# cvg/nice-slam

Measured on AMD Instinct MI355X. Metric: rendered rays/sec (fwd+bwd) per mapping iter, higher is better.
Workload: dtype f32 (f64 sample placement / depth)

## Files before the change

nice_slam_amd/build.py:

```python
from __future__ import annotations

import os
import shutil
import subprocess

HERE = os.path.dirname(os.path.abspath(__file__))
CSRC = os.path.join(HERE, "csrc")
OUT = os.path.join(HERE, "libnsr.so")
SOURCES = ("nsr_api.cpp",)
HEADERS = ("nsr_kernels.h", "nsr_recon.h", "nsr_meshdist.h", "nsr_bound.h", "nsr_raster.h", "nsr_view.h", "nsr_imgmetrics.h", "nsr_figure.h", "nsr_frame.h", "nsr_pose.h", "nsr_trajeval.h", "nsr_jpeg.h", "nsr_jpegdec.h", "nsr_bwd2.h", "nsr_fwd2.h", "nsr_layout.h", "nsr_dev.h", "nsr_rt.h", os.path.join("..", "..", "include", "nsr.h"))
FLAGS = ("--offload-arch=gfx950", "-O3", "-std=c++17", "-ffp-contract=off", "-munsafe-fp-atomics",
         "-fPIC", "-shared", "-x", "hip")


def hipcc_path() -> str:
    for cand in (os.environ.get("HIPCC"), shutil.which("hipcc"), "/opt/rocm/bin/hipcc"):
        if cand and os.path.exists(cand):
            return cand
    raise RuntimeError("hipcc not found: cannot build libnsr.so")


STAMP = os.path.join(HERE, "libnsr.srchash")


def source_hash() -> str:
    import hashlib
    h = hashlib.sha256(" ".join(FLAGS).encode())
    for f in SOURCES + HEADERS:
        with open(os.path.join(CSRC, f), "rb") as fh:
            h.update(f.encode() + b"\0" + fh.read())
    return h.hexdigest()


def is_fresh() -> bool:
    if not os.path.exists(OUT) or not os.path.exists(STAMP):
        return False
    try:
        with open(STAMP) as f:
            return f.read().strip() == source_hash()
    except OSError:
        return False


def build_lib(force: bool = False, verbose: bool = False) -> str:
    if not force and is_fresh():
        return OUT
    stamp = source_hash()
    cmd = [hipcc_path(), *FLAGS, "-Rpass-analysis=kernel-resource-usage", *[os.path.join(CSRC, s) for s in SOURCES], "-o", OUT]
    if verbose:
        print(" ".join(cmd))
    res = subprocess.run(cmd, capture_output=True, text=True)
    if res.returncode != 0:
        raise RuntimeError("hipcc failed:\n" + res.stdout + res.stderr)
    _write_resources(res.stderr)
    with open(STAMP, "w") as f:
        f.write(stamp + "\n")
    return OUT


RESOURCES = os.path.join(HERE, "libnsr.resources.json")


def _write_resources(remarks: str):
    import json
    import re
    out, name = {}, None
    for line in remarks.splitlines():
        m = re.search(r"Function Name: (\S+)", line)
        if m:
            name = m.group(1)
            out[name] = {}
            continue
        for key, pat in (("vgprs", r" VGPRs: (\d+)"), ("agprs", r"AGPRs: (\d+)"), ("scratch_bytes_per_lane", r"ScratchSize \[bytes/lane\]: (\d+)"),
                         ("sgprs", r"TotalSGPRs: (\d+)"), ("occupancy_waves_per_simd", r"Occupancy \[waves/SIMD\]: (\d+)")):
            m = re.search(pat, line)
            if m and name:
                out[name][key] = int(m.group(1))
    with open(RESOURCES, "w") as f:
        json.dump(out, f, indent=1, sort_keys=True)


if __name__ == "__main__":
    print(build_lib(force=True, verbose=True))
```

nice_slam_amd/csrc/nsr_api.cpp:

```cpp
#include <cmath>
#include <cstdio>
#include <cstdlib>
#include <cstring>
#include <map>
#include <mutex>
#include <string>
#include <utility>

#include "nsr_rt.h"
#include "nsr_kernels.h"
#include "../../nice_slam_amd/csrc/nsr_recon.h"
#include "../../nice_slam_amd/csrc/nsr_meshdist.h"
#include "../../nice_slam_amd/csrc/nsr_bound.h"
#include "../../nice_slam_amd/csrc/nsr_raster.h"
#include "../../nice_slam_amd/csrc/nsr_view.h"
#include "../../nice_slam_amd/csrc/nsr_imgmetrics.h"
#include "../../nice_slam_amd/csrc/nsr_figure.h"
#include "../../nice_slam_amd/csrc/nsr_frame.h"
#include "../../nice_slam_amd/csrc/nsr_pose.h"
#include "../../nice_slam_amd/csrc/nsr_trajeval.h"
#include "../../nice_slam_amd/csrc/nsr_jpeg.h"
#include "../../nice_slam_amd/csrc/nsr_jpegdec.h"

namespace {
// ... 127 lines not shown
    for (int s = first; s <= last; ++s) {
        const nsr_grid &g = a->grid[s];
        if (!g.feat) return fail("nsr: missing feature grid for this stage");
        if (g.Z < 1 || g.Y < 1 || g.X < 1) return fail("nsr: bad grid shape");
        if ((long long)g.Z * g.Y * g.X >= (1ll << 25)) return fail("nsr: grid too large for 32-bit byte offsets (2^25 voxels = 4 GB)");
        nsr::GridDev &G = P.grid[s];
        G.feat = g.feat; G.dfeat = g.dfeat; G.gmask = a->grad_voxel_mask[s]; G.Z = g.Z; G.Y = g.Y; G.X = g.X;
        for (int i = 0; i < 3; ++i) {
            if (!(g.hi[i] > g.lo[i])) return fail("nsr: empty normalisation box");
            G.lo[i] = g.lo[i];
            G.ext[i] = g.hi[i] - g.lo[i];
            G.inv[i] = 1.0 / (g.hi[i] - g.lo[i]);
        }
        const nsr_decoder &d = a->dec[s];
        if (!d.params || !d.packed) return fail("nsr: missing decoder parameters / packed stream for this stage");
        P.dec[s].params = d.params; P.dec[s].packed = d.packed; P.dec[s].dparams = d.dparams;
    }
    P.depth = a->depth; P.var = a->var; P.rgb = a->rgb; P.raw = a->raw; P.zvals = a->zvals;
    P.gt_color = a->gt_color; P.keep = a->keep; P.loss = a->loss; P.w_color = a->w_color;
    P.skip_masked = (a->skip_masked && a->keep && a->acts && a->zvals && a->raw) ? 1 : 0;
    P.dl_depth = a->dl_depth; P.dl_rgb = a->dl_rgb; P.loss_depth = a->gt_depth;
    return 0;
}

int finish(const char *what) {
    if (const char *e = nsr::rt_check_last()) return fail(std::string(what) + ": " + e);
    return 0;
}

template <typename K>
int launch_cfg(K kernel, int lds_bytes, const char *what) {
    if (lds_bytes > kLdsLimit) return fail(std::string(what) + ": LDS budget exceeded");
    if (lds_bytes <= 48 * 1024) return 0;
    static std::mutex mu;
    static std::map<std::pair<const void *, int>, int> granted;
    const std::pair<const void *, int> key(reinterpret_cast<const void *>(kernel), nsr::rt_current_device());
    std::lock_guard<std::mutex> lock(mu);
    int &g = granted[key];
    if (lds_bytes > g) {
        if (const char *e = nsr::rt_allow_lds(kernel, lds_bytes)) return fail(std::string(what) + ": " + e);
        g = lds_bytes;
    }
    return 0;
}

int fwd_lds_bytes(int stage, int npts) {
    const int wl = stage == NSR_STAGE_COARSE ? nsr::packed_total(0) : (stage == NSR_STAGE_MIDDLE ? nsr::packed_total(1) : nsr::packed_total(2));
    return round16(3 * nsr::AUX_FLOATS * 4) + npts * (8 + 8 + 16) + wl * 4;
}

int render_bwd_split(const nsr_render_args *a, const nsr_bwd_args *b, nsr::RenderParams &P, bool any_params, void *stream) {
    const SplitLayout L = split_layout(P.stage, P.n_rays, P.S);
    if (L.stride * 4 >= (1ll << 31)) return fail("nsr_render_bwd: more than 2^25 sample points in one call (split the ray batch)");
    const SplitGeo G = split_geo(P.stage, P.n_rays, P.S, b->max_blocks);
    const int passes = bwd_passes(P.stage);
    P.dy = P.acts + L.o_dy;
    P.draw = P.acts + L.o_draw;
    P.pf = P.acts + L.o_pf;
    P.pd = reinterpret_cast<double *>(P.acts + L.o_pd);
    for (int s = 0; s < 4; ++s)
        if (P.dec[s].dparams && (P.acts_masks_only & (1 | (2 << (s == NSR_COARSE ? 0 : s - NSR_MIDDLE)))))
            return fail("nsr_render_bwd: the forward saved relu masks only for a decoder whose parameter gradients are asked for (acts_masks_only); they need the full activations");
    if (P.dec[NSR_FINE].dparams && (P.acts_masks_only & (1 | 2)))
        return fail("nsr_render_bwd: the forward saved relu masks only for the middle decoder (acts_masks_only), whose features the fine decoder's parameter gradients read");
    if (any_params) {
        const long long need = (long long)passes * ((long long)G.nimg * P.partial_stride + (long long)G.nb * nsr::kDbPart);
        if (!b->workspace || b->workspace_floats < need) return fail("nsr_render_bwd: workspace too small");
        P.partials = b->workspace;
        P.dbpart = b->workspace + (long long)passes * G.nimg * P.partial_stride;
    }
    if (b->ev_start) nsr::rt_record(b->ev_start, stream);
    const bool draw_ready = b->loss_grads_from_forward && a->loss && a->dl_depth && b->d_depth == a->dl_depth && !b->d_var &&
                            (b->d_rgb == nullptr || b->d_rgb == a->dl_rgb) && (P.stage != NSR_STAGE_COLOR || b->d_rgb == a->dl_rgb || !a->gt_color);
    P.draw_scaled = draw_ready ? 0 : 1;
    if (!draw_ready) {
        const int tb = 256, rays_per_block = tb / 64;
        NSR_LAUNCH(nsr::comp_bwd_kernel, dim3((unsigned)((P.n_rays + rays_per_block - 1) / rays_per_block)), dim3(tb), 0, stream, P);
    }
    const bool rays = P.d_rays_o != nullptr;
    {
        int lds = 0;
        const int first = P.stage == NSR_STAGE_COARSE ? NSR_COARSE : NSR_MIDDLE, last = P.stage == NSR_STAGE_COARSE ? NSR_COARSE : P.stage;
        for (int kind = first; kind <= last; ++kind) {
            const int need = (nsr::AUX_FLOATS + nsr::packedT_total(kind) + G.waves * nsr::kDxStg + 4) * 4;
            lds = need > lds ? need : lds;
        }
        P.hot_slots = 0;
        if (P.stage != NSR_STAGE_COARSE) {
            int slots = (kLdsLimit - lds) / (nsr::kHotRow * 4);
            slots = slots > kHotSlotCap ? kHotSlotCap : slots;
            P.hot_slots = slots < 16 ? 16 : slots;
            lds += P.hot_slots * nsr::kHotRow * 4;
        }
        for (int s = 0; s < 4; ++s) {
            P.hot_z[s] = 0.f;
            if (s == NSR_COARSE || kHotCells <= 0 || !P.grid[s].dfeat) continue;
            double cell = 0.0;
            const int nn[3] = {P.grid[s].X, P.grid[s].Y, P.grid[s].Z};
            for (int ax = 0; ax < 3; ++ax) { const double c = nn[ax] > 1 ? P.grid[s].ext[ax] / (nn[ax] - 1) : 0.0; cell = c > cell ? c : cell; }
            P.hot_z[s] = (float)(kHotCells * cell);
        }
        P.lds_grid_floats = 0;
        if (P.stage == NSR_STAGE_COARSE && P.grid[NSR_COARSE].dfeat) {
            const long long gf = (long long)P.grid[NSR_COARSE].X * P.grid[NSR_COARSE].Y * P.grid[NSR_COARSE].Z * nsr::kC;
            if (lds + gf * 4 <= kLdsLimit) { P.lds_grid_floats = (int)gf; lds += (int)gf * 4; }
        }
        {
            const long long tiles = (P.n_points_total + nsr::kTile - 1) / nsr::kTile;
            int wgt[3] = {0, 0, 0}, wsum = 0;
            for (int p = 0; p < passes; ++p) {
                const int s = P.stage == NSR_STAGE_COARSE ? NSR_COARSE : NSR_MIDDLE + p;
                wgt[p] = (P.dec[s].dparams || rays || P.stage == NSR_STAGE_COARSE) ? kDxFullWeight : kDxLightWeight;
                wsum += wgt[p];
            }
            const int total = passes * G.nb;
            int used = 0;
            P.dx_beg[0] = 0;
            for (int p = 0; p < 3; ++p) {
                long long n = 0;
                if (p < passes) {
                    n = p == passes - 1 ? total - used : (long long)total * wgt[p] / wsum;
                    if (n < 1) n = 1;
                    if (n > tiles) n = tiles;
                }
                used += (int)n;
                P.dx_beg[p + 1] = P.dx_beg[p] + (int)n;
            }
        }
        const dim3 grid(P.dx_beg[3]), block(64 * G.waves);
#define NSR_DX(ST, RY)                                                                                  \
    if (int rc = launch_cfg(nsr::render_bwd_dx_kernel<ST, RY>, lds, "nsr_render_bwd(dx)")) return rc;   \
    NSR_LAUNCH((nsr::render_bwd_dx_kernel<ST, RY>), grid, block, lds, stream, P);
        switch (P.stage) {
            case 0: if (rays) { NSR_DX(0, true) } else { NSR_DX(0, false) } break;
            case 1: if (rays) { NSR_DX(1, true) } else { NSR_DX(1, false) } break;
            case 2: if (rays) { NSR_DX(2, true) } else { NSR_DX(2, false) } break;
            default: if (rays) { NSR_DX(3, true) } else { NSR_DX(3, false) } break;
        }
#undef NSR_DX
    }
    if (b->ev_dx_done) nsr::rt_record(b->ev_dx_done, stream);
    if (any_params) {
        const int lds = nsr::dw_lds_bytes(P.stage >= NSR_STAGE_FINE ? NSR_FINE : NSR_MIDDLE);
        const long long tiles = (P.n_points_total + nsr::kTile - 1) / nsr::kTile;
        int wgt[3] = {0, 0, 0}, wsum = 0;
        for (int p = 0; p < passes; ++p) {
            const int s = P.stage == NSR_STAGE_COARSE ? NSR_COARSE : NSR_MIDDLE + p;
            wgt[p] = P.dec[s].dparams ? (s == NSR_FINE ? dw_fine_weight(P.stage) : kDwWeight) : 0;
            wsum += wgt[p];
        }
        const int total = passes * G.nimg;
        P.dw_beg[0] = 0;
        for (int p = 0; p < 3; ++p) {
            long long n = (p < passes && wgt[p]) ? (long long)total * wgt[p] / wsum : 0;
            if (p < passes && wgt[p] && n < 1) n = 1;
            if (n > tiles) n = tiles;
            P.dw_beg[p + 1] = P.dw_beg[p] + (int)n;
        }
        const dim3 grid(P.dw_beg[3]), block(64 * nsr::kDwWaves);
#define NSR_DW(ST)                                                                                  \
    if (int rc = launch_cfg(nsr::render_bwd_dw_kernel<ST>, lds, "nsr_render_bwd(dw)")) return rc;   \
    NSR_LAUNCH((nsr::render_bwd_dw_kernel<ST>), grid, block, lds, stream, P);
        switch (P.stage) {
            case 0: NSR_DW(0) break;
            case 1: NSR_DW(1) break;
            case 2: NSR_DW(2) break;
            default: NSR_DW(3) break;
// ... 1987 lines not shown
```

nice_slam_amd/csrc/nsr_bwd2.h:

```cpp
#pragma once

namespace nsr {

constexpr int kDySlots = 10;
constexpr int kDxMaxWaves = 12;
constexpr int kDxTx = 0, kDxTab = kTile * kTxS, kDxP = kDxTab + 256, kDxDP = kDxP + 48, kDxStg = kDxDP + 48;
static_assert(kDxStg % 4 == 0, "staging regions must stay 16-byte aligned");
constexpr int kDbPart = 288;
NSR_KERNEL void comp_bwd_kernel(const RenderParams P) {
    const int lane = tid() & 63, wave = tid() >> 6, nw = nthreads() >> 6;
    const long long ray = (long long)bid_x() * nw + wave;
    if (ray >= P.n_rays) return;
    const int S = P.S;
    if (!ray_live(P, ray)) {
        if (lane < S) st4(P.draw + (ray * S + lane) * 4, F4{0.f, 0.f, 0.f, 0.f});
        return;
    }
    const bool act = lane < S;
    const long long gp = ray * S + (act ? lane : 0);
    const F4 rw = act ? ld4(P.raw + gp * 4) : F4{0.f, 0.f, 0.f, 0.f};
    const double sc = P.g_scale ? P.g_scale[0] : 1.0;
    const double gD = P.d_depth ? P.d_depth[ray] * sc : 0.0, gV = P.d_var ? P.d_var[ray] * sc : 0.0, dep = P.g_depth[ray];
    float gr = 0.f, gg = 0.f, gb = 0.f;
    if (P.d_rgb) { gr = P.d_rgb[ray * 3 + 0] * (float)sc; gg = P.d_rgb[ray * 3 + 1] * (float)sc; gb = P.d_rgb[ray * 3 + 2] * (float)sc; }
    const double z = act ? P.zvals[gp] : 0.0;
    const Comp cw = comp_weights(rw.w, act, lane);
    const double dz = z - dep;
    const double s1 = wave_sum_d((double)cw.w * dz);
    const float Gz = (float)(gD * z + gV * (dz * dz - 2.0 * s1 * z));
    const float Gw = Gz + fmaf(gb, rw.z, fmaf(gg, rw.y, gr * rw.x));
    float v = act ? Gw * cw.w : 0.f;
#pragma unroll
    for (int d = 1; d < 64; d <<= 1) {
        const float o = shfl_down(v, d);
        if (lane + d < 64) v += o;
    }
    float suffix = shfl_down(v, 1);
    if (lane == 63) suffix = 0.f;
    const float dalpha = Gw * cw.T - suffix / cw.t;
    float docc = 10.f * (dalpha * ((1.f - cw.alpha) * cw.alpha));
    const double px = (double)P.rays_o[ray * 3 + 0] + (double)P.rays_d[ray * 3 + 0] * z;
    const double py = (double)P.rays_o[ray * 3 + 1] + (double)P.rays_d[ray * 3 + 1] * z;
    const double pz = (double)P.rays_o[ray * 3 + 2] + (double)P.rays_d[ray * 3 + 2] * z;
    const bool inside = (px > P.blo[0]) && (px < P.bhi[0]) && (py > P.blo[1]) && (py < P.bhi[1]) && (pz > P.blo[2]) && (pz < P.bhi[2]);
    if (!inside) docc = 0.f;
    if (act) {
        st4(P.draw + gp * 4, F4{cw.w * gr, cw.w * gg, cw.w * gb, docc});
        double *q = P.pd + gp * 4;
        q[0] = px; q[1] = py; q[2] = pz; q[3] = z;
        st4(P.pf + gp * 4, F4{(float)px, (float)py, (float)pz, 0.f});
    }
}

template <int NTK>
NSR_DEV void gemv_t(f32x4 (&dx)[NTK], const Act<2> &dy, const float *wt, int lane) {
#pragma unroll
    for (int To = 0; To < 2; ++To) {
        f32x4 a[NTK];
#pragma unroll
        for (int Tk = 0; Tk < NTK; ++Tk) a[Tk] = to_v(ld4(wt + ((Tk * 2 + To) * 64 + lane) * 4));
#pragma unroll
        for (int r = 0; r < 4; ++r)
#pragma unroll
            for (int Tk = 0; Tk < NTK; ++Tk) dx[Tk] = mfma16(a[Tk][r], dy.t[To][r], dx[Tk]);
    }
    sched_fence();
}

struct DxIn {
    F4 dr;
    unsigned m0, m1;
};
NSR_DEV DxIn dx_load(const RenderParams &P, const float *acts_pass, long long tile, int pt, int g) {
    DxIn I;
    const long long gp = tile * kTile + pt;
    const long long q = gp < P.n_points_total ? gp : 0;
    I.dr = ld4(P.draw + q * 4);
    const float *mp = acts_pass + ((q >> 4) * kActSlots + kActMask) * 256 + ((q & 15) * 4 + g) * 4;
    I.m0 = __builtin_bit_cast(unsigned, mp[0]);
    I.m1 = __builtin_bit_cast(unsigned, mp[1]);
    return I;
}
NSR_DEV void dx_keep(const DxIn &I) {
    keep_alive(I.dr.w); keep_alive(__builtin_bit_cast(float, I.m1));
}

template <int KIND, bool PARAMS, bool RAYS>
NSR_DEV void dx_pass(const RenderParams &P, int bi, int nbp, int gb) {
    constexpr bool XYZ = KIND != NSR_COARSE;
    constexpr int NOUT = nout_of(KIND);
    char *lds = lds_base();
    const int lane = tid() & 63, wave = uniform(tid() >> 6), nw = nthreads() >> 6;
    const int pt = lane & 15, g = lane >> 4;
    float *aux = reinterpret_cast<float *>(lds);
    float *wt = aux + AUX_FLOATS;
    float *stg = wt + packedT_total(KIND);
    float *Sw = stg + wave * kDxStg;
    const int tail_off = uniform((int)(stg + nw * kDxStg - reinterpret_cast<float *>(lds)));
    const int gl_off = (KIND == NSR_COARSE && P.lds_grid_floats > 0) ? tail_off : -1;
    float *gl = gl_off >= 0 ? reinterpret_cast<float *>(lds) + gl_off : nullptr;
    const bool use_hot = KIND != NSR_COARSE && P.hot_z[KIND] > 0.f && P.grid[KIND].dfeat != nullptr;
    const HotTab hot{use_hot ? tail_off : -1, P.hot_slots};
    int *tcnt = reinterpret_cast<int *>(stg + nw * kDxStg + (KIND == NSR_COARSE ? P.lds_grid_floats : P.hot_slots * kHotRow));
    const GridDev &G = P.grid[KIND];
    const DecDev &D = P.dec[KIND];
    const bool do_grid = G.dfeat != nullptr;
    if (!do_grid && !PARAMS && !RAYS) return;
    const Dbg dbg{P.dbg ? P.dbg + ((long long)gb * kDxMaxWaves + wave) * 64 : nullptr};
    dbg.stamp(0);
    constexpr long long sstride = 256;
    const float *acts_pass = P.acts + (long long)act_pass(KIND) * P.act_tiles * kActSlots * 256;
    const long long ntiles = (P.n_points_total + kTile - 1) / kTile;
    const long long t0 = ntiles * bi / nbp, tend = ntiles * (bi + 1) / nbp;
    long long tile = t0 + wave;
    const bool pre = tile < tend && tile_live(P, tile);
    DxIn cur;
    if (pre) cur = dx_load(P, acts_pass, tile, pt, g);
    copy_f4<AUX_FLOATS / 4>(aux, D.packed);
    copy_f4_dma<packedT_total(KIND) / 4>(wt, D.packed + AUX_FLOATS + packed_total(KIND));
    if (gl) for (int i = tid(); i < P.lds_grid_floats; i += nthreads()) gl[i] = 0.f;
    if (use_hot) hot_init(hot);
    if (tid() == 0) tcnt[0] = nw;
    dma_wait<0>();
    block_sync();
    dbg.stamp(1);
    float *dys = P.dy + (long long)act_pass(KIND) * P.act_tiles * kDySlots * 256;
    const bool need_dc = do_grid || RAYS;
    float aB[kET][3];
#pragma unroll
    for (int k = 0; k < kET; ++k) { aB[k][0] = 0.f; aB[k][1] = 0.f; aB[k][2] = 0.f; }

    auto claim = [&]() -> long long {
        for (;;) {
            int k = 0;
            if (lane == 0) k = atomic_fetch_add_lds_i(tcnt, 1);
            const long long t = t0 + shfl_i(k, 0);
            if (t >= tend || tile_live(P, t)) return t;
        }
    };
    const float dr_scale = (!P.draw_scaled && P.g_scale) ? (float)P.g_scale[0] : 1.f;
    if (!pre) {
        tile = claim();
        if (tile < tend) cur = dx_load(P, acts_pass, tile, pt, g);
    }
    if (tile < tend) dx_keep(cur);
    while (tile < tend) {
        loop_fence();
        const long long nxt = claim();
        const bool has_next = nxt < tend;
        DxIn nx = cur;
        if (has_next) nx = dx_load(P, acts_pass, nxt, pt, g);
        const long long gp = tile * kTile + pt;
        const bool active = gp < P.n_points_total;
        const double *pp = P.pd + (active ? gp : 0) * 4;
        const double cpx = pp[0], cpy = pp[1], cpz = pp[2], cz = pp[3];
        dbg.stamp(2);
        const unsigned mw0 = active ? cur.m0 : 0u, mw1 = active ? cur.m1 : 0u;
        const float dsc = active ? dr_scale : 0.f;
        float d_out[4] = {0.f, 0.f, 0.f, 0.f};
        if (NOUT == 1) d_out[0] = cur.dr.w * dsc;
        else { d_out[0] = cur.dr.x * dsc; d_out[1] = cur.dr.y * dsc; d_out[2] = cur.dr.z * dsc; }
        Act<2> dh;
#pragma unroll
        for (int T = 0; T < 2; ++T) {
            f32x4 v = f4zero();
#pragma unroll
            for (int n = 0; n < (NOUT == 1 ? 1 : 3); ++n) {
                const F4 w = ld4(aux + AUX_WO + n * 32 + 16 * T + 4 * g);
                v[0] = fmaf(w.x, d_out[n], v[0]); v[1] = fmaf(w.y, d_out[n], v[1]);
                v[2] = fmaf(w.z, d_out[n], v[2]); v[3] = fmaf(w.w, d_out[n], v[3]);
            }
            dh.t[T] = v;
        }
        Act<2> dc, dY0, dY3;
        act_zero(dc); act_zero(dY0); act_zero(dY3);
        float *dyp = dys + tile * (kDySlots * 256) + (pt * 4 + g) * 4;
#pragma unroll
        for (int I = 4; I >= 0; --I) {
            if (XYZ && need_dc) gemv_t<2>(dc.t, dh, wt + xyzT_u(I), lane);
            const Act<2> dY = apply_mask(dh, I < 4 ? mw0 : mw1, I < 4 ? 8 * I : 0);
            if (PARAMS && active) {
                st4(dyp + (2 * I) * sstride, to_F4(dY.t[0]));
                st4(dyp + (2 * I + 1) * sstride, to_F4(dY.t[1]));
            }
            if (I == 3) dY3 = dY;
            if (I == 0) dY0 = dY;
            if (!XYZ) {
                if (I == 3 && need_dc) gemv_t<2>(dc.t, dY, wt + nox_mat(NW3C).pk, lane);
                if (I == 0 && need_dc) gemv_t<2>(dc.t, dY, wt + nox_mat(NW0).pk, lane);
            }
            if (I > 0) {
                Act<2> nd;
                act_zero(nd);
                if (XYZ) gemv_t<2>(nd.t, dY, wt + xyzT_wh(I - 1), lane);
                else gemv_t<2>(nd.t, dY, wt + nox_mat(I == 1 ? NW1 : (I == 2 ? NW2 : (I == 3 ? NW3H : NW4))).pk, lane);
                dh = nd;
            }
        }
        dbg.stamp(3);
        const float px = (float)cpx, py = (float)cpy, pz = (float)cpz;
        float dpe[3] = {0.f, 0.f, 0.f};
        if (XYZ && PARAMS && ballot64(active) != 0ull) {
            if (g == 0) { Sw[kDxP + pt] = px; Sw[kDxP + 16 + pt] = py; Sw[kDxP + 32 + pt] = pz; }
            wave_fence();
            const f32x4 qx = to_v(ld4(Sw + kDxP + 4 * g)), qy = to_v(ld4(Sw + kDxP + 16 + 4 * g)), qz = to_v(ld4(Sw + kDxP + 32 + 4 * g));
            f32x4 sx = f4zero(), sy = f4zero(), sz = f4zero();
#pragma unroll
            for (int Tk = 0; Tk < kET; ++Tk) {
                f32x4 e0 = f4zero(), e3 = f4zero();
#pragma unroll
                for (int To = 0; To < 2; ++To) {
                    const f32x4 a0 = to_v(ld4(wt + xyzT_w0() + ((Tk * 2 + To) * 64 + lane) * 4));
                    const f32x4 a3 = to_v(ld4(wt + xyzT_w3e() + ((Tk * 2 + To) * 64 + lane) * 4));
#pragma unroll
                    for (int r = 0; r < 4; ++r) {
                        e0 = mfma16(dY0.t[To][r], a0[r], e0);
                        e3 = mfma16(dY3.t[To][r], a3[r], e3);
                    }
                }
                sched_fence();
                const F4 b = load_b1(aux, 16 * Tk + pt);
                const f32x4 darg = (e0 + e3) * cos_dx4(vfma(qz, splat(b.z), vfma(qy, splat(b.y), qx * splat(b.x))));
#pragma unroll
                for (int r = 0; r < 4; ++r) {
                    aB[Tk][0] = fmaf(darg[r], qx[r], aB[Tk][0]); aB[Tk][1] = fmaf(darg[r], qy[r], aB[Tk][1]);
                    aB[Tk][2] = fmaf(darg[r], qz[r], aB[Tk][2]);
                }
                if (RAYS) { sx = vfma(darg, splat(b.x), sx); sy = vfma(darg, splat(b.y), sy); sz = vfma(darg, splat(b.z), sz); }
            }
            if (RAYS) {
#pragma unroll
                for (int m = 1; m < 16; m <<= 1)
#pragma unroll
                    for (int r = 0; r < 4; ++r) { sx[r] += shfl_xor(sx[r], m); sy[r] += shfl_xor(sy[r], m); sz[r] += shfl_xor(sz[r], m); }
                if (pt == 0) { st4(Sw + kDxDP + 4 * g, to_F4(sx)); st4(Sw + kDxDP + 16 + 4 * g, to_F4(sy)); st4(Sw + kDxDP + 32 + 4 * g, to_F4(sz)); }
                wave_fence();
                dpe[0] = Sw[kDxDP + pt]; dpe[1] = Sw[kDxDP + 16 + pt]; dpe[2] = Sw[kDxDP + 32 + pt];
            }
            wave_fence();
        } else if (XYZ && RAYS) {
            f32x4 dE[kET];
#pragma unroll
            for (int Tk = 0; Tk < kET; ++Tk) dE[Tk] = f4zero();
            gemv_t<kET>(dE, dY0, wt + xyzT_w0(), lane);
            gemv_t<kET>(dE, dY3, wt + xyzT_w3e(), lane);
            float ax = 0.f, ay = 0.f, az = 0.f;
#pragma unroll
            for (int Tk = 0; Tk < kET; ++Tk) {
                const B4 b = load_b4(aux, 4 * Tk + g);
                const f32x4 darg = dE[Tk] * cos_dx4(vfma(splat(pz), b.z, vfma(splat(py), b.y, splat(px) * b.x)));
#pragma unroll
                for (int r = 0; r < 4; ++r) { ax = fmaf(darg[r], b.x[r], ax); ay = fmaf(darg[r], b.y[r], ay); az = fmaf(darg[r], b.z[r], az); }
                sched_fence();
            }
            dpe[0] = red_g(ax); dpe[1] = red_g(ay); dpe[2] = red_g(az);
        }
        dbg.stamp(4);
        Lvl L;
        if (need_dc) L = make_level(G, cpx, cpy, cpz);
        const unsigned live = (do_grid && G.gmask) ? gmask_bits(G, L, g) : 3u;
        float dux = 0.f, duy = 0.f, duz = 0.f;
        if (RAYS) coord_grad(G, L, g, dc, dux, duy, duz);
        dx_keep(nx);
        keep_alive_d(cpx); keep_alive_d(cpy); keep_alive_d(cpz); keep_alive_d(cz);
        dbg.stamp(5);
        if (do_grid)
            scatter_merged(G, L, lane, dc, active, Sw + kDxTx, Sw + kDxTab, gl_off, hot, (float)cz < P.hot_z[KIND], live);
        dbg.stamp(6);
        if (RAYS) {
            double v[6];
            const bool mine = active && g == 0;
            v[0] = mine ? (double)dux * (2.0 * G.inv[0]) + (double)dpe[0] : 0.0;
            v[1] = mine ? (double)duy * (2.0 * G.inv[1]) + (double)dpe[1] : 0.0;
            v[2] = mine ? (double)duz * (2.0 * G.inv[2]) + (double)dpe[2] : 0.0;
            v[3] = v[0] * cz; v[4] = v[1] * cz; v[5] = v[2] * cz;
            if ((P.S & (kTile - 1)) == 0) {
#pragma unroll
                for (int m = 1; m < 16; m <<= 1)
#pragma unroll
                    for (int q = 0; q < 6; ++q) v[q] += shfl_xor_d(v[q], m);
                if (lane == 0 && active) {
                    const long long ray = (long long)((unsigned)gp / (unsigned)P.S);
#pragma unroll
                    for (int q = 0; q < 3; ++q) {
                        atomic_add_global(P.d_rays_o + ray * 3 + q, (float)v[q]);
                        atomic_add_global(P.d_rays_d + ray * 3 + q, (float)v[3 + q]);
                    }
                }
            } else if (mine) {
                const long long ray = (long long)((unsigned)gp / (unsigned)P.S);
#pragma unroll
                for (int q = 0; q < 3; ++q) {
                    atomic_add_global(P.d_rays_o + ray * 3 + q, (float)v[q]);
                    atomic_add_global(P.d_rays_d + ray * 3 + q, (float)v[3 + q]);
                }
            }
        }
        cur = nx;
        tile = nxt;
        dbg.stamp(7);
    }
    dbg.stamp(8);
    if (XYZ && PARAMS) {
#pragma unroll
        for (int k = 0; k < kET; ++k)
#pragma unroll
            for (int d = 0; d < 3; ++d) {
                float v = aB[k][d];
                v += shfl_xor(v, 16); v += shfl_xor(v, 32);
                if (g == 0) Sw[d * 96 + 16 * k + pt] = v;
            }
    }
    if (use_hot || (gl && do_grid) || (XYZ && PARAMS)) block_sync();
    dbg.stamp(10);
    if (XYZ && PARAMS) {
        float *part = P.dbpart + (long long)gb * kDbPart;
        for (int t = tid(); t < kDbPart; t += nthreads()) {
            float s = 0.f;
            for (int w = 0; w < nw; ++w) s += stg[w * kDxStg + t];
            part[t] = s;
        }
    }
    if (use_hot) hot_flush(hot, G);
    dbg.stamp(11);
    if (gl && do_grid) {
        for (int i = tid(); i < P.lds_grid_floats; i += nthreads()) {
            const float v = gl[i];
            if (v != 0.f) atomic_add_global(G.dfeat + i, v);
// ... 595 lines not shown
```

nice_slam_amd/csrc/nsr_kernels.h:

```cpp
#pragma once
#include "nsr_dev.h"
#include "nsr_layout.h"
#include "../../include/nsr.h"

namespace nsr {

template <int NT>
struct Act { f32x4 t[NT]; };

NSR_DEV f32x4 f4zero() { f32x4 v = {0.f, 0.f, 0.f, 0.f}; return v; }
NSR_DEV f32x4 to_v(F4 a) { f32x4 v = {a.x, a.y, a.z, a.w}; return v; }
NSR_DEV F4 to_F4(f32x4 v) { return F4{v[0], v[1], v[2], v[3]}; }
template <int NT> NSR_DEV void act_zero(Act<NT> &a) {
#pragma unroll
    for (int T = 0; T < NT; ++T) a.t[T] = f4zero();
}

NSR_DEV double tmax(double a, double b) { return (a > b || a != a) ? a : b; }
NSR_DEV double tmin(double a, double b) { return (a < b || a != a) ? a : b; }

struct GridDev {
    const float *feat;
    float *dfeat;
    const unsigned char *gmask;
    int Z, Y, X;
    double lo[3];
    double ext[3];
    double inv[3];
};

struct DecDev {
    const float *params;
    const float *packed;
    float *dparams;
};

struct RenderParams {
    int stage, n_samples, n_surface, S;
    long long n_rays;
    int rays_per_block, tiles_per_block;
    long long n_groups;
    const float *rays_o, *rays_d, *gt_depth, *gt_max;
    double blo[3], bhi[3];
    float t_uniform[NSR_MAX_SAMPLES];
    double t_surface[NSR_MAX_SAMPLES];
    GridDev grid[4];
    DecDev dec[4];
    double *depth, *var;
    float *rgb, *raw;
    double *zvals;
    float *acts;
    int acts_masks_only;
    long long n_points_total;
    long long act_tiles;
    const double *d_depth, *d_var, *g_depth;
    const double *g_scale;
    const float *d_rgb;
    float *d_rays_o, *d_rays_d;
    float *partials;
    int partial_stride;
    const float *loss_depth;
    const float *gt_color;
    const unsigned char *keep;
    double *loss;
    double *dl_depth;
    float *dl_rgb;
    float w_color;
    long long *dbg;
    float *dy;
    float *draw;
    double *pd;
    float *pf;
    float *dbpart;
    int dw_beg[4];
    int dx_beg[4];
    int draw_scaled;
    int skip_masked;
    int lds_grid_floats;
    float hot_z[4];
    int hot_slots;
    unsigned s_magic;
    int pass_beg[4];
    const double *points;
    long long n_points;
    float *out_points;
// ... 1979 lines not shown
```

nice_slam_amd/csrc/nsr_layout.h:

```cpp
#pragma once

namespace nsr {

constexpr int kC = 32;
constexpr int kH = 32;
constexpr int kE = 93;
constexpr int kET = 6;
constexpr int kTile = 16;
constexpr int kTxS = 36;

struct Mat {
    int off;
    int stride;
    int kbeg;
    int kcols;
    int nt;
    int pk;
};

constexpr int cdim_of(int kind) { return kind == 2 ? 64 : 32; }
constexpr int nout_of(int kind) { return kind == 3 ? 4 : 1; }
constexpr bool is_xyz(int kind) { return kind != 0; }

constexpr int xyz_fcw(int cd, int i) { return i * (32 * cd + 32); }
// ... 17 lines not shown
}
constexpr int xyz_pk(int cd, int id) {
    int o = 0;
    for (int j = 0; j < id; ++j) o += xyz_nt(cd, j) * 512;
    return o;
}
constexpr Mat xyz_mat(int cd, int id) {
    switch (id) {
        case XW0: return Mat{xyz_w(cd, 0), kE, 0, kE, kET, xyz_pk(cd, id)};
        case XU0: return Mat{xyz_fcw(cd, 0), cd, 0, cd, cd / 16, xyz_pk(cd, id)};
        case XW1: return Mat{xyz_w(cd, 1), 32, 0, 32, 2, xyz_pk(cd, id)};
        case XU1: return Mat{xyz_fcw(cd, 1), cd, 0, cd, cd / 16, xyz_pk(cd, id)};
        case XW2: return Mat{xyz_w(cd, 2), 32, 0, 32, 2, xyz_pk(cd, id)};
        case XU2: return Mat{xyz_fcw(cd, 2), cd, 0, cd, cd / 16, xyz_pk(cd, id)};
        case XW3E: return Mat{xyz_w(cd, 3), kE + 32, 0, kE, kET, xyz_pk(cd, id)};
        case XW3H: return Mat{xyz_w(cd, 3), kE + 32, kE, 32, 2, xyz_pk(cd, id)};
        case XU3: return Mat{xyz_fcw(cd, 3), cd, 0, cd, cd / 16, xyz_pk(cd, id)};
        case XW4: return Mat{xyz_w(cd, 4), 32, 0, 32, 2, xyz_pk(cd, id)};
        default: return Mat{xyz_fcw(cd, 4), cd, 0, cd, cd / 16, xyz_pk(cd, id)};
    }
}
constexpr int xyz_packed_total(int cd) { return xyz_pk(cd, XNMAT); }

constexpr int nox_in(int i) { return i == 3 ? 64 : 32; }
constexpr int nox_w(int i) {
    int o = 0;
    for (int j = 0; j < i; ++j) o += 32 * nox_in(j) + 32;
    return o;
}
constexpr int nox_b(int i) { return nox_w(i) + 32 * nox_in(i); }
constexpr int nox_wo() { return nox_b(4) + 32; }
constexpr int nox_bo() { return nox_wo() + 32; }
constexpr int nox_total() { return nox_bo() + 1; }
enum { NW0 = 0, NW1 = 1, NW2 = 2, NW3C = 3, NW3H = 4, NW4 = 5, NNMAT = 6 };
constexpr Mat nox_mat(int id) {
    switch (id) {
        case NW0: return Mat{nox_w(0), 32, 0, 32, 2, 0};
        case NW1: return Mat{nox_w(1), 32, 0, 32, 2, 1024};
        case NW2: return Mat{nox_w(2), 32, 0, 32, 2, 2048};
        case NW3C: return Mat{nox_w(3), 64, 0, 32, 2, 3072};
        case NW3H: return Mat{nox_w(3), 64, 32, 32, 2, 4096};
        default: return Mat{nox_w(4), 32, 0, 32, 2, 5120};
    }
}
constexpr int nox_packed_total() { return 6144; }

constexpr int param_total(int kind) { return kind == 0 ? nox_total() : xyz_total(cdim_of(kind), nout_of(kind)); }
constexpr int packed_total(int kind) { return kind == 0 ? nox_packed_total() : xyz_packed_total(cdim_of(kind)); }
constexpr int nmat_of(int kind) { return kind == 0 ? (int)NNMAT : (int)XNMAT; }
constexpr Mat mat_of(int kind, int id) { return kind == 0 ? nox_mat(id) : xyz_mat(cdim_of(kind), id); }
constexpr int bias_off(int kind, int i) { return kind == 0 ? nox_b(i) : xyz_b(cdim_of(kind), i); }
constexpr int fcb_off(int kind, int i) { return xyz_fcb(cdim_of(kind), i); }
constexpr int wo_off(int kind) { return kind == 0 ? nox_wo() : xyz_wo(cdim_of(kind)); }
constexpr int bo_off(int kind) { return kind == 0 ? nox_bo() : xyz_bo(cdim_of(kind), nout_of(kind)); }
constexpr int B_off(int kind) { return xyz_B(cdim_of(kind)); }

static_assert(param_total(0) == 6337, "coarse decoder parameter count");
static_assert(param_total(1) == 15800, "middle decoder parameter count");
static_assert(param_total(2) == 20920, "fine decoder parameter count");
static_assert(param_total(3) == 15899, "color decoder parameter count");

constexpr int AUX_B = 0;
constexpr int AUX_V = 160;
constexpr int AUX_WO = 320;
constexpr int AUX_BO = 448;
constexpr int AUX_BM = 452;
constexpr int AUX_FLOATS = 452 + 96 * 4;
constexpr int xyzT_u(int i) { return i * 1024; }
constexpr int xyzT_wh(int m) { return 5120 + m * 1024; }
constexpr int xyzT_w0() { return 9216; }
constexpr int xyzT_w3e() { return 12288; }
constexpr int xyzT_total() { return 15360; }
constexpr int packedT_total(int kind) { return kind == 0 ? nox_packed_total() : xyzT_total(); }
constexpr int xyzT_nmat() { return 11; }
constexpr Mat xyzT_mat(int cd, int id) {
    return id < 5 ? Mat{xyz_fcw(cd, id), cd, 0, 32, 2, xyzT_u(id)}
         : id == 5 ? Mat{xyz_w(cd, 1), 32, 0, 32, 2, xyzT_wh(0)}
         : id == 6 ? Mat{xyz_w(cd, 2), 32, 0, 32, 2, xyzT_wh(1)}
         : id == 7 ? Mat{xyz_w(cd, 3), kE + 32, kE, 32, 2, xyzT_wh(2)}
         : id == 8 ? Mat{xyz_w(cd, 4), 32, 0, 32, 2, xyzT_wh(3)}
         : id == 9 ? Mat{xyz_w(cd, 0), kE, 0, kE, kET, xyzT_w0()}
                   : Mat{xyz_w(cd, 3), kE + 32, 0, kE, kET, xyzT_w3e()};
}
constexpr int nmatT_of(int kind) { return kind == 0 ? (int)NNMAT : xyzT_nmat(); }
constexpr Mat matT_of(int kind, int id) { return kind == 0 ? nox_mat(id) : xyzT_mat(cdim_of(kind), id); }

constexpr int packed_buf_total(int kind) { return AUX_FLOATS + packed_total(kind) + packedT_total(kind); }
static_assert(AUX_FLOATS % 4 == 0, "the operand stream behind the aux table must stay 16-byte aligned");

}
```

Measured before the change: 4.758 million.

## Use split-bf16 MFMA for embedding-gradient products in dx backward

```diff
diff --git a/nice_slam_amd/build.py b/nice_slam_amd/build.py
--- a/nice_slam_amd/build.py
+++ b/nice_slam_amd/build.py
@@ -8,7 +8,7 @@
 CSRC = os.path.join(HERE, "csrc")
 OUT = os.path.join(HERE, "libnsr.so")
 SOURCES = ("nsr_api.cpp",)
-HEADERS = ("nsr_kernels.h", "nsr_recon.h", "nsr_meshdist.h", "nsr_bound.h", "nsr_raster.h", "nsr_view.h", "nsr_imgmetrics.h", "nsr_figure.h", "nsr_frame.h", "nsr_pose.h", "nsr_trajeval.h", "nsr_jpeg.h", "nsr_jpegdec.h", "nsr_bwd2.h", "nsr_fwd2.h", "nsr_layout.h", "nsr_dev.h", "nsr_rt.h", os.path.join("..", "..", "include", "nsr.h"))
+HEADERS = ("nsr_kernels.h", "nsr_recon.h", "nsr_meshdist.h", "nsr_bound.h", "nsr_raster.h", "nsr_view.h", "nsr_imgmetrics.h", "nsr_figure.h", "nsr_frame.h", "nsr_pose.h", "nsr_trajeval.h", "nsr_jpeg.h", "nsr_jpegdec.h", "nsr_bwd2.h", "nsr_fwd2.h", "nsr_layout.h", "nsr_split.h", "nsr_dev.h", "nsr_rt.h", os.path.join("..", "..", "include", "nsr.h"))
 FLAGS = ("--offload-arch=gfx950", "-O3", "-std=c++17", "-ffp-contract=off", "-munsafe-fp-atomics",
          "-fPIC", "-shared", "-x", "hip")
 
diff --git a/nice_slam_amd/csrc/nsr_api.cpp b/nice_slam_amd/csrc/nsr_api.cpp
--- a/nice_slam_amd/csrc/nsr_api.cpp
+++ b/nice_slam_amd/csrc/nsr_api.cpp
@@ -233,7 +233,7 @@
         int lds = 0;
         const int first = P.stage == NSR_STAGE_COARSE ? NSR_COARSE : NSR_MIDDLE, last = P.stage == NSR_STAGE_COARSE ? NSR_COARSE : P.stage;
         for (int kind = first; kind <= last; ++kind) {
-            const int need = (nsr::AUX_FLOATS + nsr::packedT_total(kind) + G.waves * nsr::kDxStg + 4) * 4;
+            const int need = (nsr::AUX_FLOATS + nsr::dx_stream_lds(kind) + G.waves * nsr::kDxStg + 4) * 4;
             lds = need > lds ? need : lds;
         }
         P.hot_slots = 0;
diff --git a/nice_slam_amd/csrc/nsr_bwd2.h b/nice_slam_amd/csrc/nsr_bwd2.h
--- a/nice_slam_amd/csrc/nsr_bwd2.h
+++ b/nice_slam_amd/csrc/nsr_bwd2.h
@@ -66,6 +66,19 @@
     }
     sched_fence();
 }
+NSR_DEV bf16x8w ld_plane(const float *p) {
+    const F4 v = ld4(p);
+    bf16x8w w = {__builtin_bit_cast(unsigned, v.x), __builtin_bit_cast(unsigned, v.y), __builtin_bit_cast(unsigned, v.z), __builtin_bit_cast(unsigned, v.w)};
+    return w;
+}
+NSR_DEV void st_plane(float *p, bf16x8w w) {
+    const unsigned w0 = w[0], w1 = w[1], w2 = w[2], w3 = w[3];
+    st4(p, F4{__builtin_bit_cast(float, w0), __builtin_bit_cast(float, w1), __builtin_bit_cast(float, w2), __builtin_bit_cast(float, w3)});
+}
+NSR_DEV Bf3 ld_planes(const float *planes, int Tk, int lane) {
+    const float *p = planes + (Tk * 3 * 64 + lane) * 4;
+    return Bf3{ld_plane(p), ld_plane(p + 256), ld_plane(p + 512)};
+}
 
 struct DxIn {
     F4 dr;
@@ -94,7 +107,7 @@
     const int pt = lane & 15, g = lane >> 4;
     float *aux = reinterpret_cast<float *>(lds);
     float *wt = aux + AUX_FLOATS;
-    float *stg = wt + packedT_total(KIND);
+    float *stg = wt + dx_stream_lds(KIND);
     float *Sw = stg + wave * kDxStg;
     const int tail_off = uniform((int)(stg + nw * kDxStg - reinterpret_cast<float *>(lds)));
     const int gl_off = (KIND == NSR_COARSE && P.lds_grid_floats > 0) ? tail_off : -1;
@@ -116,11 +129,27 @@
     const bool pre = tile < tend && tile_live(P, tile);
     DxIn cur;
     if (pre) cur = dx_load(P, acts_pass, tile, pt, g);
+    const float *streamT = D.packed + AUX_FLOATS + packed_total(KIND);
+    constexpr bool EMB = XYZ && (PARAMS || RAYS);
+    constexpr int kPlaneJobs = 2 * kET * 64;
+    int pj = tid();
+    F4 pv0 = F4{0.f, 0.f, 0.f, 0.f}, pv1 = pv0;
+    auto plane_src = [&](int j) { return streamT + (j >= kET * 64 ? xyzT_w3e() : xyzT_w0()) + (((j >> 6) % kET) * 128 + (j & 63)) * 4; };
+    if (EMB && pj < kPlaneJobs) { pv0 = ld4(plane_src(pj)); pv1 = ld4(plane_src(pj) + 256); }
     copy_f4<AUX_FLOATS / 4>(aux, D.packed);
-    copy_f4_dma<packedT_total(KIND) / 4>(wt, D.packed + AUX_FLOATS + packed_total(KIND));
+    copy_f4_dma<(XYZ ? xyzT_copied() : packedT_total(KIND)) / 4>(wt, streamT);
     if (gl) for (int i = tid(); i < P.lds_grid_floats; i += nthreads()) gl[i] = 0.f;
     if (use_hot) hot_init(hot);
     if (tid() == 0) tcnt[0] = nw;
+    if (EMB) {
+        while (pj < kPlaneJobs) {
+            const Bf3 s = split_pack8(to_v(pv0), to_v(pv1));
+            float *dst = wt + xyzL_planes(pj >= kET * 64 ? 1 : 0) + (((pj >> 6) % kET) * 3 * 64 + (pj & 63)) * 4;
+            st_plane(dst, s.hi); st_plane(dst + 256, s.mid); st_plane(dst + 512, s.lo);
+            pj += nthreads();
+            if (pj < kPlaneJobs) { pv0 = ld4(plane_src(pj)); pv1 = ld4(plane_src(pj) + 256); }
+        }
+    }
     dma_wait<0>();
     block_sync();
     dbg.stamp(1);
@@ -203,22 +232,21 @@
         if (XYZ && PARAMS && ballot64(active) != 0ull) {
             if (g == 0) { Sw[kDxP + pt] = px; Sw[kDxP + 16 + pt] = py; Sw[kDxP + 32 + pt] = pz; }
             wave_fence();
-            const f32x4 qx = to_v(ld4(Sw + kDxP + 4 * g)), qy = to_v(ld4(Sw + kDxP + 16 + 4 * g)), qz = to_v(ld4(Sw + kDxP + 32 + 4 * g));
             f32x4 sx = f4zero(), sy = f4zero(), sz = f4zero();
+            static_assert(3 * 256 <= kDxP, "dY3's planes fit in front of the staged positions");
+            const Bf3 y0 = split_pack8(dY0.t[0], dY0.t[1]);
+            {
+                const Bf3 y3 = split_pack8(dY3.t[0], dY3.t[1]);
+                st_plane(Sw + lane * 4, y3.hi); st_plane(Sw + 256 + lane * 4, y3.mid); st_plane(Sw + 512 + lane * 4, y3.lo);
+            }
 #pragma unroll
             for (int Tk = 0; Tk < kET; ++Tk) {
-                f32x4 e0 = f4zero(), e3 = f4zero();
-#pragma unroll
-                for (int To = 0; To < 2; ++To) {
-                    const f32x4 a0 = to_v(ld4(wt + xyzT_w0() + ((Tk * 2 + To) * 64 + lane) * 4));
-                    const f32x4 a3 = to_v(ld4(wt + xyzT_w3e() + ((Tk * 2 + To) * 64 + lane) * 4));
-#pragma unroll
-                    for (int r = 0; r < 4; ++r) {
-                        e0 = mfma16(dY0.t[To][r], a0[r], e0);
-                        e3 = mfma16(dY3.t[To][r], a3[r], e3);
-                    }
-                }
+                loop_fence();
+                const f32x4 e0 = mfma16_split3(y0, ld_planes(wt + xyzL_planes(0), Tk, lane), f4zero());
                 sched_fence();
+                const f32x4 e3 = mfma16_split3(ld_planes(Sw, 0, lane), ld_planes(wt + xyzL_planes(1), Tk, lane), f4zero());
+                sched_fence();
+                const f32x4 qx = to_v(ld4(Sw + kDxP + 4 * g)), qy = to_v(ld4(Sw + kDxP + 16 + 4 * g)), qz = to_v(ld4(Sw + kDxP + 32 + 4 * g));
                 const F4 b = load_b1(aux, 16 * Tk + pt);
                 const f32x4 darg = (e0 + e3) * cos_dx4(vfma(qz, splat(b.z), vfma(qy, splat(b.y), qx * splat(b.x))));
 #pragma unroll
@@ -227,6 +255,7 @@
                     aB[Tk][2] = fmaf(darg[r], qz[r], aB[Tk][2]);
                 }
                 if (RAYS) { sx = vfma(darg, splat(b.x), sx); sy = vfma(darg, splat(b.y), sy); sz = vfma(darg, splat(b.z), sz); }
+                keep_alive(aB[Tk][0]); keep_alive(aB[Tk][1]); keep_alive(aB[Tk][2]);
             }
             if (RAYS) {
 #pragma unroll
@@ -238,12 +267,20 @@
                 dpe[0] = Sw[kDxDP + pt]; dpe[1] = Sw[kDxDP + 16 + pt]; dpe[2] = Sw[kDxDP + 32 + pt];
             }
             wave_fence();
-        } else if (XYZ && RAYS) {
+        } else if (XYZ && RAYS && !PARAMS && ballot64(active) != 0ull) {
             f32x4 dE[kET];
 #pragma unroll
             for (int Tk = 0; Tk < kET; ++Tk) dE[Tk] = f4zero();
-            gemv_t<kET>(dE, dY0, wt + xyzT_w0(), lane);
-            gemv_t<kET>(dE, dY3, wt + xyzT_w3e(), lane);
+#pragma unroll
+            for (int m = 0; m < 2; ++m) {
+                const Bf3 y = m ? split_pack8(dY3.t[0], dY3.t[1]) : split_pack8(dY0.t[0], dY0.t[1]);
+#pragma unroll
+                for (int Tk = 0; Tk < kET; Tk += 2) {
+                    dE[Tk] = mfma16_split3(ld_planes(wt + xyzL_planes(m), Tk, lane), y, dE[Tk]);
+                    dE[Tk + 1] = mfma16_split3(ld_planes(wt + xyzL_planes(m), Tk + 1, lane), y, dE[Tk + 1]);
+                    sched_fence();
+                }
+            }
             float ax = 0.f, ay = 0.f, az = 0.f;
 #pragma unroll
             for (int Tk = 0; Tk < kET; ++Tk) {
diff --git a/nice_slam_amd/csrc/nsr_kernels.h b/nice_slam_amd/csrc/nsr_kernels.h
--- a/nice_slam_amd/csrc/nsr_kernels.h
+++ b/nice_slam_amd/csrc/nsr_kernels.h
@@ -1,6 +1,7 @@
 #pragma once
 #include "nsr_dev.h"
 #include "nsr_layout.h"
+#include "../../nice_slam_amd/csrc/nsr_split.h"
 #include "../../include/nsr.h"
 
 namespace nsr {
diff --git a/nice_slam_amd/csrc/nsr_layout.h b/nice_slam_amd/csrc/nsr_layout.h
--- a/nice_slam_amd/csrc/nsr_layout.h
+++ b/nice_slam_amd/csrc/nsr_layout.h
@@ -123,6 +123,10 @@
          : id == 9 ? Mat{xyz_w(cd, 0), kE, 0, kE, kET, xyzT_w0()}
                    : Mat{xyz_w(cd, 3), kE + 32, 0, kE, kET, xyzT_w3e()};
 }
+constexpr int xyzT_copied() { return xyzT_w0(); }
+constexpr int xyzL_planes(int m) { return xyzT_w0() + m * (kET * 3 * 256); }
+constexpr int xyzL_total() { return xyzL_planes(2); }
+constexpr int dx_stream_lds(int kind) { return kind == 0 ? nox_packed_total() : xyzL_total(); }
 constexpr int nmatT_of(int kind) { return kind == 0 ? (int)NNMAT : xyzT_nmat(); }
 constexpr Mat matT_of(int kind, int id) { return kind == 0 ? nox_mat(id) : xyzT_mat(cdim_of(kind), id); }
 
diff --git a/nice_slam_amd/csrc/nsr_split.h b/nice_slam_amd/csrc/nsr_split.h
--- /dev/null
+++ b/nice_slam_amd/csrc/nsr_split.h
@@ -0,0 +1,73 @@
+#pragma once
+
+namespace nsr {
+
+typedef float s3_f32x4 __attribute__((ext_vector_type(4)));
+typedef unsigned bf16x8w __attribute__((ext_vector_type(4)));
+
+struct Split3 { unsigned hi, mid, lo; };
+NSR_DEV Split3 split3(float x) {
+    const unsigned hb = __builtin_bit_cast(unsigned, x) & 0xffff0000u;
+    const float r = x - __builtin_bit_cast(float, hb);
+    const unsigned mb = __builtin_bit_cast(unsigned, r) & 0xffff0000u;
+    const float l = r - __builtin_bit_cast(float, mb);
+    return Split3{hb, mb, __builtin_bit_cast(unsigned, l)};
+}
+NSR_DEV unsigned pack_bf16x2(unsigned even, unsigned odd) { return (even >> 16) | (odd & 0xffff0000u); }
+
+struct Bf3 { bf16x8w hi, mid, lo; };
+NSR_DEV Bf3 split_pack8(s3_f32x4 t0, s3_f32x4 t1) {
+    Bf3 o;
+#pragma unroll
+    for (int d = 0; d < 4; ++d) {
+        const s3_f32x4 &t = d < 2 ? t0 : t1;
+        const Split3 a = split3(t[2 * (d & 1)]), b = split3(t[2 * (d & 1) + 1]);
+        o.hi[d] = pack_bf16x2(a.hi, b.hi); o.mid[d] = pack_bf16x2(a.mid, b.mid); o.lo[d] = pack_bf16x2(a.lo, b.lo);
+    }
+    return o;
+}
+
+#ifndef NSR_SPLIT_SCALAR_ONLY
+#if defined(__HIP_DEVICE_COMPILE__)
+typedef __bf16 s3_bf16x8 __attribute__((ext_vector_type(8)));
+NSR_DEV s3_f32x4 mfma16_bf16(bf16x8w a, bf16x8w b, s3_f32x4 c) {
+    return __builtin_amdgcn_mfma_f32_16x16x32_bf16(__builtin_bit_cast(s3_bf16x8, a), __builtin_bit_cast(s3_bf16x8, b), c, 0, 0, 0);
+}
+#else
+NSR_DEV float bf16_half(unsigned w, int half) { return __builtin_bit_cast(float, half ? (w & 0xffff0000u) : (w << 16)); }
+NSR_DEV s3_f32x4 mfma16_bf16(bf16x8w a, bf16x8w b, s3_f32x4 c) {
+    const int lane = tid() & 63, col = lane & 15, g = lane >> 4;
+    unsigned bw[16];
+#pragma unroll
+    for (int kg = 0; kg < 4; ++kg)
+#pragma unroll
+        for (int d = 0; d < 4; ++d) bw[4 * kg + d] = (unsigned)shfl_i((int)b[d], col + 16 * kg);
+    s3_f32x4 out = c;
+#pragma unroll
+    for (int r = 0; r < 4; ++r) {
+        float s = c[r];
+#pragma unroll
+        for (int kg = 0; kg < 4; ++kg)
+#pragma unroll
+            for (int d = 0; d < 4; ++d) {
+                const unsigned aw = (unsigned)shfl_i((int)a[d], 4 * g + r + 16 * kg);
+                s += bf16_half(aw, 0) * bf16_half(bw[4 * kg + d], 0);
+                s += bf16_half(aw, 1) * bf16_half(bw[4 * kg + d], 1);
+            }
+        out[r] = s;
+    }
+    return out;
+}
+#endif
+NSR_DEV s3_f32x4 mfma16_split3(const Bf3 &a, const Bf3 &b, s3_f32x4 c) {
+    c = mfma16_bf16(a.hi, b.lo, c);
+    c = mfma16_bf16(a.lo, b.hi, c);
+    c = mfma16_bf16(a.mid, b.mid, c);
+    c = mfma16_bf16(a.hi, b.mid, c);
+    c = mfma16_bf16(a.mid, b.hi, c);
+    c = mfma16_bf16(a.hi, b.hi, c);
+    return c;
+}
+#endif
+
+}
```

Measured after the change: 4.639 million. 2.5% lower.
